# geekuillaume/node-speex-resampler

Hardware: AMD Instinct MI355X
Metric: input Msamples/s int16 44100->48000 q=7 2ch (whole job) (higher is better)
Workload: dtype f32

## Files before the change

### node-speex-resampler_amd/csrc/gen_fir_loop.py

```python
#!/usr/bin/env python3
import os

BANKS = {
    (10, 2): dict(A=[(28, 4), (36, 16)], B=[(52, 16), (68, 4)]),
    (5, 6): dict(A=[(4, 16), (20, 8), (28, 4), (36, 2)], B=[(40, 16), (56, 8), (64, 4), (38, 2)]),
    (5, 4): dict(A=[(28, 4), (36, 16)], B=[(52, 16), (68, 4)]),
}
SAMPLE_BASE = {10: 40, 5: 64}


def tap_reg(bank, t):
    for first, n in bank:
        if t < n:
            return first + t
        t -= n
    raise ValueError(t)


def bank_regs(bank):
    return [r for first, n in bank for r in range(first, first + n)]


class Variant:
    def __init__(self, R, S, CT, CF, padded, w16):
# ... 16 lines not shown
    def fma_bank(self, which, lo, hi):
        bank = self.banks[which]
        out = []
        for u in range(self.S):
            k = u if which == "A" else self.S + u
            for i in range(lo, hi):
                r = tap_reg(bank, u * self.R + i)
                h = r & 1
                p = r - h
                out.append("v_pk_fma_f32 %%[a%d], s[%d:%d], v[%d:%d], %%[a%d] op_sel:[%d,0,0] op_sel_hi:[%d,1,1]"
                           % (i, p, p + 1, self.pair(k), self.pair(k) + 1, i, h, h))
        return out

    def tap_loads(self, which, byte_off):
        out, t = [], 0
        for f, m in self.banks[which]:
            out.append("s_load_dword%s s[%d:%d], %%[rows], %%[off] offset:0x%x"
                       % ("x%d" % m if m > 1 else "", f, f + m - 1, byte_off + 4 * t))
            t += m
        return out

    def sample_reads(self, which, first_step):
        out = []
        if self.CT == 2 and not self.w16 and self.S % 2 == 0 and os.environ.get("SPEEXHIP_GEN_READ2"):
            for u in range(0, self.S, 2):
                k = u if which == "A" else self.S + u
                o0 = (first_step + u) * self.CF * 4 // 8
                o1 = (first_step + u + 1) * self.CF * 4 // 8
                p = self.pair(k)
                out.append("ds_read2_b64 v[%d:%d], %%[addr] offset0:%d offset1:%d" % (p, p + 3, o0, o1))
            return out
        for u in range(self.S):
            k = u if which == "A" else self.S + u
            o = (first_step + u) * self.CF * self.eb
            p = self.pair(k)
            if self.CT == 2 and not self.w16:
                out.append("ds_read_b64 v[%d:%d], %%[addr] offset:%d" % (p, p + 1, o))
            elif self.CT == 2:
                out.append("ds_read_b32 v%d, %%[addr] offset:%d" % (self.raw(k), o))
            elif not self.w16:
                out += ["ds_read_b32 v%d, %%[addr] offset:%d" % (p, o), "ds_read_b32 v%d, %%[addr2] offset:%d" % (p + 1, o)]
            else:
                out += ["ds_read_i16 v%d, %%[addr] offset:%d" % (p, o), "ds_read_i16 v%d, %%[addr2] offset:%d" % (p + 1, o)]
        return out

    def converts(self, which):
        if not self.w16:
            return []
        out = []
        for u in range(self.S):
            k = u if which == "A" else self.S + u
            p = self.pair(k)
            if self.CT == 2:
                out += ["v_cvt_f32_i32_sdwa v%d, sext(v%d) dst_sel:DWORD dst_unused:UNUSED_PAD src0_sel:WORD_0" % (p, self.raw(k)),
                        "v_cvt_f32_i32_sdwa v%d, sext(v%d) dst_sel:DWORD dst_unused:UNUSED_PAD src0_sel:WORD_1" % (p + 1, self.raw(k))]
            else:
                out += ["v_cvt_f32_i32_e32 v%d, v%d" % (p, p), "v_cvt_f32_i32_e32 v%d, v%d" % (p + 1, p + 1)]
        return out

    def loop(self, label, cnt, lo, hi):
        S, R = self.S, self.R
        bank_bytes = 4 * S * R
        adv = 2 * S * self.CF * self.eb
        body = ["s_sub_u32 %%[%s], %%[%s], 1" % (cnt, cnt), "s_cbranch_scc1 %d1f" % label, "%d0:" % label]
        body += ["s_waitcnt lgkmcnt(0)"] + self.tap_loads("B", bank_bytes) + self.sample_reads("B", S)
        body += self.converts("A") + self.fma_bank("A", lo, hi)
        body += ["s_waitcnt lgkmcnt(0)"]
        if self.padded:
            body += ["s_sub_u32 %[wrap], %[wrap], 1", "s_cmp_eq_u32 %[wrap], 0",
                     "s_cselect_b32 %[tmp], %[advpad], " + str(adv), "s_cselect_b32 %[wrap], %[wrapstep], %[wrap]",
                     "v_add_u32 %[addr], %[tmp], %[addr]"]
            if self.CT == 1:
                body += ["v_add_u32 %[addr2], %[tmp], %[addr2]"]
        else:
            body += ["v_add_u32 %%[addr], %d, %%[addr]" % adv]
            if self.CT == 1:
                body += ["v_add_u32 %%[addr2], %d, %%[addr2]" % adv]
        body += self.tap_loads("A", 2 * bank_bytes) + self.sample_reads("A", 0)
        body += self.converts("B") + self.fma_bank("B", lo, hi)
        body += ["s_add_u32 %%[off], %%[off], 0x%x" % (2 * bank_bytes), "s_sub_u32 %%[%s], %%[%s], 1" % (cnt, cnt),
                 "s_cbranch_scc0 %d0b" % label, "%d1:" % label]
        return body

    def lines(self):
        pro = self.tap_loads("A", 0) + self.sample_reads("A", 0)
        if self.R == 10:
            body = self.loop(1, "head", 0, 5) + self.loop(2, "main", 0, 10) + self.loop(3, "tail", 5, 10)
        else:
            body = self.loop(2, "main", 0, self.R)
        return pro + body + ["s_waitcnt lgkmcnt(0)"]

    def function(self):
        R = self.R
        asm = "\n".join('      "%s\\n"' % l for l in self.lines())
        outs = ['[a%d] "+v"(acc[%d])' % (i, i) for i in range(R)] + ['[addr] "+v"(addr)']
        if self.CT == 1:
            outs.append('[addr2] "+v"(addr2)')
        outs += ['[off] "+s"(off)', '[main] "+s"(main)']
        if R == 10:
            outs += ['[head] "+s"(head)', '[tail] "+s"(tail)']
        ins = ['[rows] "s"(rows_g)']
        if self.padded:
            outs += ['[wrap] "+s"(to_wrap)', '[tmp] "=&s"(tmp)']
            ins += ['[advpad] "s"(adv_pad)', '[wrapstep] "s"(wrap_step)']
        clob = ['"s%d"' % r for r in bank_regs(self.banks["A"]) + bank_regs(self.banks["B"])] + ['"v%d"' % r for r in self.vgprs()]
        return '''template <>
struct FirLoopAsm<%d, %d, %d, %s, %s> {
  static constexpr bool available = true;
  static constexpr int steps_per_bank = %d;
  // rows_g: the group's tap rows; addr / addr2: LDS byte addresses of the lane's first sample (second period);
  // head / main / tail: trips on rows [0, R/2) / all rows / rows [R/2, R); to_wrap, wrap_step: trips to the
  // first / between period boundaries of a padded window, adv_pad: window bytes per trip + the padding
  static __device__ __forceinline__ void run(f32x2 (&acc)[%d], const float *rows_g, uint32_t addr, uint32_t addr2,
                                             uint32_t head, uint32_t main, uint32_t tail, uint32_t to_wrap,
                                             uint32_t wrap_step, uint32_t adv_pad) {
    uint32_t off = 0, tmp;
    (void)tmp; (void)addr2; (void)head; (void)tail; (void)to_wrap; (void)wrap_step; (void)adv_pad;
    asm volatile(
%s
      : %s
      : %s
      : %s, "scc", "memory");
  }
};
''' % (R, self.CT, self.CF, "true" if self.padded else "false", "true" if self.w16 else "false", self.S, R, asm,
       ", ".join(outs), ", ".join(ins), ", ".join(clob))


class Variant64(Variant):

    def __init__(self, R, S, CT, CF, padded, w16=False):
        Variant.__init__(self, R, 2 * S, CT, CF, padded, False)
        self.S = S
        self.vbase = {10: 56, 5: 64}[R]
        self.w16 = w16
        self.eb = 2 if w16 else 4
        self.name = "A64_R%d_S%d_CT%d_CF%d_P%d_W%d" % (R, S, CT, CF, int(padded), int(w16))

    def quad(self, k):
        return self.vbase + 4 * k

    def vgprs(self):
        return list(range(self.vbase, self.vbase + 8 * self.S))

    def tap_pair(self, which, t):
        r = tap_reg(self.banks[which], 2 * t)
        assert r % 2 == 0 and tap_reg(self.banks[which], 2 * t + 1) == r + 1
        return r

    def fma_bank(self, which, lo, hi):
        out = []
        for u in range(self.S):
            k = u if which == "A" else self.S + u
            q = self.quad(k)
            for i in range(lo, hi):
                r = self.tap_pair(which, u * self.R + i)
                out.append("v_fma_f64 %%[a%dx], s[%d:%d], v[%d:%d], %%[a%dx]" % (i, r, r + 1, q, q + 1, i))
                out.append("v_fma_f64 %%[a%dy], s[%d:%d], v[%d:%d], %%[a%dy]" % (i, r, r + 1, q + 2, q + 3, i))
        return out

    def tap_loads(self, which, byte_off):
        out, t = [], 0
        for f, m in self.banks[which]:
            out.append("s_load_dword%s s[%d:%d], %%[rows], %%[off] offset:0x%x"
                       % ("x%d" % m if m > 1 else "", f, f + m - 1, byte_off + 4 * t))
            t += m
        return out

    def sample_reads(self, which, first_step):
        out = []
        for u in range(self.S):
            k = u if which == "A" else self.S + u
            o = (first_step + u) * self.CF * self.eb
# ... 144 lines not shown
        body += ["s_waitcnt lgkmcnt(0)"]
        if self.padded:
            body += ["s_sub_u32 %[wrap], %[wrap], 1", "s_cmp_eq_u32 %[wrap], 0",
                     "s_cselect_b32 %[tmp], %[advpad], " + str(adv), "s_cselect_b32 %[wrap], %[wrapstep], %[wrap]",
                     "v_add_u32 %[addr], %[tmp], %[addr]"]
        else:
            body += ["v_add_u32 %%[addr], %d, %%[addr]" % adv]
        body += self.tap_loads("A", 2 * bank_bytes) + self.sample_reads("A", 0)
        body += self.converts("B") + self.fma_bank("B", lo, hi)
        body += ["s_add_u32 %%[off], %%[off], 0x%x" % (2 * bank_bytes), "s_sub_u32 %%[%s], %%[%s], 1" % (cnt, cnt),
                 "s_cbranch_scc0 %d0b" % label, "%d1:" % label]
        return body

    def function(self):
        R = self.R
        asm = "\n".join('      "%s\\n"' % l for l in self.lines())
        outs = ['[a%d] "+v"(acc[%d])' % (i, i) for i in range(R)] + ['[addr] "+v"(addr)']
        outs += ['[off] "+s"(off)', '[main] "+s"(main)']
        if R == 10:
            outs += ['[head] "+s"(head)', '[tail] "+s"(tail)']
        ins = ['[rows] "s"(rows_g)']
        if self.padded:
            outs += ['[wrap] "+s"(to_wrap)', '[tmp] "=&s"(tmp)']
            ins += ['[advpad] "s"(adv_pad)', '[wrapstep] "s"(wrap_step)']
        clob = ['"s%d"' % r for r in bank_regs(self.banks["A"]) + bank_regs(self.banks["B"])] + ['"v%d"' % r for r in self.vgprs()]
        return '''template <>
struct FirLoopAsmPP<%d, %d, %s, %s> {
  static constexpr bool available = true;
  static constexpr int steps_per_bank = %d;
  // as FirLoopAsm::run; acc[i] = phases 2i and 2i + 1 of the lane's period; rows_g: [trip][step][2R] floats
  static __device__ __forceinline__ void run(f32x2 (&acc)[%d], const float *rows_g, uint32_t addr, uint32_t head, uint32_t main,
                                             uint32_t tail, uint32_t to_wrap, uint32_t wrap_step, uint32_t adv_pad) {
    uint32_t off = 0, tmp;
    (void)tmp; (void)head; (void)tail; (void)to_wrap; (void)wrap_step; (void)adv_pad;
    asm volatile(
%s
      : %s
      : %s
      : %s, "scc", "memory");
  }
};
''' % (R, self.CF, "true" if self.padded else "false", "true" if self.w16 else "false", self.S, R, asm,
       ", ".join(outs), ", ".join(ins), ", ".join(clob))

    def lines(self):
        pro = self.tap_loads("A", 0) + self.sample_reads("A", 0)
        if self.R == 10:
            body = self.loop(1, "head", 0, 5) + self.loop(2, "main", 0, 10) + self.loop(3, "tail", 5, 10)
        else:
            body = self.loop(2, "main", 0, self.R)
        return pro + body + ["s_waitcnt lgkmcnt(0)"]


def variants_pp():
    out = []
    for CF in (1, 2, 3):
        for w16 in (False, True):
            for padded in (False, True):
                out.append(VariantPP(10, 1, CF, padded, w16))
            out.append(VariantPP(5, R5_STEPS // 2, CF, False, w16))
    return out


def variants64():
    out = []
    for w16 in (False, True):
        for CT, CF in ((2, 2), (2, 4), (2, 6), (2, 8), (1, 1), (1, 3), (1, 5), (1, 7)):
            for padded in (False, True):
                out.append(Variant64(10, 1, CT, CF, padded, w16))
            out.append(Variant64(5, R5_STEPS // 2, CT, CF, False, w16))
    return out


def variants():
    out = []
    for w16 in (False, True):
        for CT, CF in ((2, 2), (2, 4), (2, 6), (2, 8), (1, 1), (1, 3), (1, 5), (1, 7), (2, 10), (2, 12), (2, 16)):
            for padded in (False, True):
                out.append(Variant(10, 2, CT, CF, padded, w16))
            out.append(Variant(5, R5_STEPS, CT, CF, False, w16))
    return out


R5_STEPS = 6

HEAD = '''// csrc/fir_loop_asm.inc -- GENERATED by csrc/gen_fir_loop.py; do not edit (see that file for the why and the how).
// The FIR inner loop of the period kernel as gfx950 ISA, one specialisation per (phases per wave, channels
// per lane, floats per frame, padded window, int16 window).  Included by kernels_period.hip only.

// primary template: no ISA variant for this layout -> fir_group runs its C++ loop
template <int R, int CT, int CF, bool PADDED, bool W16>
struct FirLoopAsm {
  static constexpr bool available = false;
};

'''


HEAD64 = '''
// ---- fp64 accumulator (round 4; gen_fir_loop.py, Variant64) ----
template <int R, int CT, int CF, bool PADDED, bool W16 = false>
struct FirLoopAsm64 {
  static constexpr bool available = false;
};

'''


HEADPP = '''
// ---- phase pairs: lane = (period, channel), two phases per packed FMA (round 4; gen_fir_loop.py, VariantPP) ----
template <int R, int CF, bool PADDED, bool W16>
struct FirLoopAsmPP {
  static constexpr bool available = false;
};

'''


def main():
    src = (HEAD + "\n".join(v.function() for v in variants()) + HEAD64 + "\n".join(v.function() for v in variants64()) +
           HEADPP + "\n".join(v.function() for v in variants_pp()))
    path = os.path.join(os.path.dirname(os.path.abspath(__file__)), "fir_loop_asm.inc")
    open(path, "w").write(src)
    print("wrote %s: %d + %d + %d variants, %d lines" % (path, len(variants()), len(variants64()), len(variants_pp()), src.count("\n")))


if __name__ == "__main__":
    main()
```

### node-speex-resampler_amd/csrc/kernels_period_impl.h

```cpp
#pragma once
#include <hip/hip_runtime.h>

#include <algorithm>
#include <cmath>
#include <cstdio>
#include <cstdlib>
#include <cstring>
#include <type_traits>
#include <vector>

#include "device_helpers.h"
#include "device_types.h"
#include "filter_design.h"
#include "kernels.h"

namespace speexhip {
#ifdef SPEEXHIP_STAMPS
static __device__ unsigned long long g_stamps[8192 * 16];
#define STAMP(k)                                                                                         \
  do {                                                                                                   \
    const uint32_t lin_ = blockIdx.x + gridDim.x * (blockIdx.y + gridDim.y * blockIdx.z);                \
    if ((threadIdx.x & 63u) == 0 && lin_ < 8192)                                                         \
      atomicMax(&g_stamps[lin_ * 16 + (k)], (unsigned long long)__builtin_amdgcn_s_memrealtime());        \
  } while (0)
#define STAMP_FIRST(k)                                                                                   \
  do {                                                                                                   \
    const uint32_t lin_ = blockIdx.x + gridDim.x * (blockIdx.y + gridDim.y * blockIdx.z);                \
    if ((threadIdx.x & 63u) == 0 && lin_ < 8192)                                                         \
      atomicMax(&g_stamps[lin_ * 16 + (k)], ~(unsigned long long)__builtin_amdgcn_s_memrealtime());       \
  } while (0)
#else
#define STAMP(k) do { } while (0)
#define STAMP_FIRST(k) do { } while (0)
#endif
namespace {

typedef float f32x2 __attribute__((ext_vector_type(2)));
__host__ __device__ constexpr int bank_taps(int r) { return r == 10 ? 20 : 30; }
typedef uint32_t u32x4_a4 __attribute__((ext_vector_type(4), aligned(4)));
typedef uint32_t u32x2_a4 __attribute__((ext_vector_type(2), aligned(4)));
typedef __attribute__((address_space(1))) u32x4_a4 g_u32x4_a4;
typedef __attribute__((address_space(1))) u32x2_a4 g_u32x2_a4;
typedef float f32x4_a4 __attribute__((ext_vector_type(4), aligned(4)));
typedef float f32x2_a4 __attribute__((ext_vector_type(2), aligned(4)));

__device__ __forceinline__ void fma_tap(f32x2 &acc, const f32x2 &tap_pair, const f32x2 &x, bool hi) {
  if (hi)
    asm("v_pk_fma_f32 %0, %1, %2, %0 op_sel:[1,0,0] op_sel_hi:[1,1,1]" : "+v"(acc) : "s"(tap_pair), "v"(x));
  else
    asm("v_pk_fma_f32 %0, %1, %2, %0 op_sel:[0,0,0] op_sel_hi:[0,1,1]" : "+v"(acc) : "s"(tap_pair), "v"(x));
}

#include "fir_loop_asm.inc"

__device__ __forceinline__ void set_fir_priority(const PeriodParams &p) {
  if (p.prio & 4u) {
    const uint32_t tg_id = (__builtin_amdgcn_s_getreg(4 | (16 << 6) | (3 << 11)));
    if (tg_id & 1u) {
      __builtin_amdgcn_s_setprio(1);
      return;
    }
  }
  __builtin_amdgcn_s_setprio(0);
}

struct LaneCtx {
  uint32_t C;
  uint32_t cg;
  bool live;
  bool live_b;
  uint32_t xlane;
  uint64_t K_lane;
};

template <int CT, bool ONE_GROUP, bool PADDED, int CGF = 0, bool PP = false, bool ROWS = false>
__device__ __forceinline__ LaneCtx lane_ctx(const PeriodParams &p, uint32_t xshift, uint32_t m_lo,
                                            uint32_t m_cnt, uint32_t lane) {
  constexpr uint32_t kGroups = ONE_GROUP ? 1u : static_cast<uint32_t>(CGF);
  const uint32_t cgroups = kGroups != 0 ? kGroups : p.cgroups;
  LaneCtx c;
  c.C = kGroups != 0 ? kGroups * CT : p.channels;
  static_assert(!ROWS || (CGF == 4 && CT == 2), "the row mapping is for frames of four channel pairs");
  c.cg = ONE_GROUP ? 0 : ROWS ? lane >> 4 : lane % cgroups;
  const uint32_t pl = ONE_GROUP ? lane : ROWS ? (lane & 15u) : lane / cgroups;
  const uint32_t lane_max = (CT == 1 && !PP) ? p.half_periods : p.lane_periods;
  c.live = pl < lane_max && pl < m_cnt;
  c.live_b = CT == 1 && !PP && pl < lane_max && pl + p.half_periods < m_cnt;
  c.xlane = xshift + min(pl, lane_max - 1) * (p.num * c.C + (PADDED ? p.pad : 0u)) + c.cg * CT;
  c.K_lane = static_cast<uint64_t>(m_lo + pl) * p.den;
  return c;
}

template <int R, int CT, bool PADDED, int CF = 0, bool W16 = false>
__device__ __forceinline__ void fir_group(const PeriodParams &p, const float *__restrict__ rows, const float *xs,
                                          const LaneCtx &c, uint32_t g, bool skip_all, f32x2 (&acc)[R]) {
  const uint32_t C = c.C;
  const uint32_t delta_g = p.delta[g];
  using E = typename std::conditional<W16, int16_t, float>::type;
  const E *xp = reinterpret_cast<const E *>(xs) + c.xlane + delta_g * C;
#ifndef SPEEXHIP_CXX_FIR_LOOP
  constexpr bool kIsa16 = W16 && CF != 0 && FirLoopAsm<R, CT, CF, PADDED, W16>::available;
#else
  constexpr bool kIsa16 = false;
#endif
  if constexpr (kIsa16) {
    using Isa = FirLoopAsm<R, CT, CF, PADDED, true>;
    constexpr uint32_t kStepsPerTrip = 2 * Isa::steps_per_bank;
    const uint32_t trips = skip_all ? 0u : p.delta[2 * p.groups + g];
    const uint32_t head = R == 10 ? trips & 15u : 0u, tail = R == 10 ? (trips >> 4) & 15u : 0u;
    const float *rows_g = rows + static_cast<size_t>(g) * p.l4 * (2 * bank_taps(R));
    const uint32_t addr = static_cast<uint32_t>(reinterpret_cast<uintptr_t>(xs)) + (c.xlane + delta_g * C) * 2u;
    auto sgpr = [](uint32_t v) { return static_cast<uint32_t>(__builtin_amdgcn_readfirstlane(static_cast<int>(v))); };
    const uint64_t rows_bits = reinterpret_cast<uint64_t>(rows_g);
    const float *rows_s = reinterpret_cast<const float *>(static_cast<uint64_t>(sgpr(static_cast<uint32_t>(rows_bits))) |
                                                          static_cast<uint64_t>(sgpr(static_cast<uint32_t>(rows_bits >> 32))) << 32);
    Isa::run(acc, rows_s, addr, CT == 1 ? addr + p.half_offset * 2u : 0u, sgpr(head), sgpr((trips >> 8) - head - tail),
             sgpr(tail), sgpr(PADDED ? p.delta[p.groups + g] : 0u), sgpr(p.wrap_step),
             sgpr((kStepsPerTrip * CF + p.pad) * 2u));
    return;
  }
#ifndef SPEEXHIP_CXX_FIR_LOOP
  using Isa = FirLoopAsm<R, CT, CF, PADDED, false>;
  if constexpr (!W16 && CF != 0 && Isa::available) {
    constexpr uint32_t kStepsPerTrip = 2 * Isa::steps_per_bank;
    static_assert(kStepsPerTrip * R == 2 * bank_taps(R), "the ISA loop and the tap rows disagree on the trip");
    const uint32_t trips = skip_all ? 0u : p.delta[2 * p.groups + g];
    const uint32_t head = R == 10 ? trips & 15u : 0u, tail = R == 10 ? (trips >> 4) & 15u : 0u;
    const float *rows_g = rows + static_cast<size_t>(g) * p.l4 * (2 * bank_taps(R));
    const uint32_t addr = static_cast<uint32_t>(reinterpret_cast<uintptr_t>(xp));
    auto sgpr = [](uint32_t v) { return static_cast<uint32_t>(__builtin_amdgcn_readfirstlane(static_cast<int>(v))); };
    const uint64_t rows_bits = reinterpret_cast<uint64_t>(rows_g);
    const float *rows_s = reinterpret_cast<const float *>(static_cast<uint64_t>(sgpr(static_cast<uint32_t>(rows_bits))) |
                                                          static_cast<uint64_t>(sgpr(static_cast<uint32_t>(rows_bits >> 32))) << 32);
    Isa::run(acc, rows_s, addr, CT == 1 ? addr + p.half_offset * 4u : 0u, sgpr(head), sgpr((trips >> 8) - head - tail),
             sgpr(tail), sgpr(PADDED ? p.delta[p.groups + g] : 0u), sgpr(p.wrap_step),
             sgpr((kStepsPerTrip * CF + p.pad) * 4u));
// ... 502 lines not shown
  auto params = [&]() -> PeriodParams {
    if constexpr (kReload) return load_k(pp);
    return p0;
  };
  constexpr bool kRows = PADDED && CGF == 4 && !W16 && AM == 0;
  const LaneCtx c = lane_ctx<CT, ONE_GROUP, PADDED, CGF, AM == 2, kRows>(p0, xshift, m_lo, m_cnt, lane);
  const uint32_t g_step = p0.wave_groups * nsplit;
  uint32_t g = zsplit * p0.wave_groups + wave;
  if (g >= p0.groups) return;
  PeriodParams p = p0;
  for (;;) {
    f32x2 acc[R];
#pragma unroll
    for (int i = 0; i < R; i++) acc[i] = f32x2{0.f, 0.f};
#ifdef SPEEXHIP_STAMPS
    const unsigned long long fir_t0 = __builtin_amdgcn_s_memtime(), fir_r0 = __builtin_amdgcn_s_memrealtime();
#endif
    if constexpr (AM == 2) {
      fir_group_pp<R, ONE_GROUP ? 1 : CGF, PADDED, W16>(p, rows, xs, c, g, SPEEXHIP_DIAG_SKIP(p, 4u), 0u, 1u, acc);
    } else if constexpr (AM == 1) {
      double acc64[R][2];
#pragma unroll
      for (int i = 0; i < R; i++) acc64[i][0] = acc64[i][1] = 0.0;
      fir_group64<R, CT, PADDED, ONE_GROUP ? CT : CT * CGF, W16>(p, reinterpret_cast<const double *>(rows), xs, c, g,
                                                                SPEEXHIP_DIAG_SKIP(p, 4u), 0u, 1u, acc64);
#pragma unroll
      for (int i = 0; i < R; i++) acc[i] = f32x2{static_cast<float>(acc64[i][0]), static_cast<float>(acc64[i][1])};
    } else {
      fir_group<R, CT, PADDED, ONE_GROUP ? CT : CT * CGF, W16>(p, rows, xs, c, g, SPEEXHIP_DIAG_SKIP(p, 4u), acc);
    }
#ifdef SPEEXHIP_STAMPS
    {
      asm volatile("" ::"v"(acc[0]));
      const unsigned long long fir_t1 = __builtin_amdgcn_s_memtime(), fir_r1 = __builtin_amdgcn_s_memrealtime();
      const uint32_t lin_ = blockIdx.x + gridDim.x * (blockIdx.y + gridDim.y * blockIdx.z);
      if ((threadIdx.x & 63u) == 0 && lin_ < 8192) atomicMax(&g_stamps[lin_ * 16 + 7], fir_t1 - fir_t0);
      if (threadIdx.x == 0 && lin_ < 8192) {
        g_stamps[lin_ * 16 + 9] = fir_t1 - fir_t0;
        g_stamps[lin_ * 16 + 10] = fir_r1 - fir_r0;
      }
    }
#endif
    STAMP(5);
    const PeriodParams q = params();
    if constexpr (kRows && sizeof(T) == 2 && R == 10) {
      if (!SPEEXHIP_DIAG_SKIP(q, 8u)) {
        StreamDesc d;
        if constexpr (kReload)
          d = load_k(dp);
        else
          d = d0;
        if (q.prio & 2u) __builtin_amdgcn_s_setprio(2);
        store_group_rows<R>(q, d, c, g, c.live, acc);
        if (q.prio & 2u) set_fir_priority(q);
        STAMP(6);
      }
    } else if (!SPEEXHIP_DIAG_SKIP(q, 8u) && c.live) {
      StreamDesc d;
      if constexpr (kReload)
        d = load_k(dp);
      else
        d = d0;
      if (q.prio & 2u) __builtin_amdgcn_s_setprio(2);
      if constexpr (AM == 2)
        store_group_pp<R, ONE_GROUP ? 1 : CGF, T>(q, d, c, g, acc);
      else
        store_group<R, CT, ONE_GROUP, T>(q, d, c, g, acc);
      if (q.prio & 2u) set_fir_priority(q);
      STAMP(6);
    }
    g += g_step;
    if (g >= q.groups) return;
    p = q;
  }
}

template <typename T>
struct StagedImage {
  static constexpr uint32_t kRowDwords = 16 * 5 * (sizeof(T) == 4 ? 2 : 1) + 1;
  static constexpr uint32_t kBytes = 64 * kRowDwords * 4;
  static constexpr uint32_t kAt = (kStagedLdsBytes - kBytes) / 16 * 16;
};

template <int R, int CT, typename T>
__device__ __forceinline__ void fir_tile_staged(const PeriodParams &p0, KParams pp, const float *__restrict__ rows, KDesc dp,
                                                float *xs, uint32_t xshift, uint32_t m_lo, uint32_t m_cnt, uint32_t wave,
                                                uint32_t lane, uint32_t zsplit) {
  static_assert(R == 5 && CT == 2, "written for stereo groups of five phases");
  using Img = StagedImage<T>;
  constexpr uint32_t kDpf = sizeof(T) == 4 ? 2u : 1u;
  uint32_t *img = reinterpret_cast<uint32_t *>(reinterpret_cast<char *>(xs) + Img::kAt);
  const uint32_t g = zsplit * p0.wave_groups + wave;
  if (wave < p0.wave_groups && g < p0.groups) {
    const LaneCtx c = lane_ctx<CT, true, false>(p0, xshift, m_lo, m_cnt, lane);
    f32x2 acc[R];
#pragma unroll
    for (int i = 0; i < R; i++) acc[i] = f32x2{0.f, 0.f};
    fir_group<R, CT, false, CT, false>(p0, rows, xs, c, g, SPEEXHIP_DIAG_SKIP(p0, 4u), acc);
    uint32_t *row = img + lane * Img::kRowDwords + wave * (R * kDpf);
#pragma unroll
    for (int i = 0; i < R; i++) {
      if constexpr (sizeof(T) == 4) {
        row[2 * i] = __float_as_uint(acc[i].x);
        row[2 * i + 1] = __float_as_uint(acc[i].y);
      } else {
        row[i] = round_pack_pcm(acc[i].x, acc[i].y);
      }
    }
  }
  __syncthreads();
  const PeriodParams q = load_k(pp);
  const StreamDesc d = load_k(dp);
  if (SPEEXHIP_DIAG_SKIP(q, 8u)) return;
  if (q.prio & 2u) __builtin_amdgcn_s_setprio(2);
  constexpr uint32_t kFb = 4u * kDpf;
  const uint32_t ph_lo = zsplit * q.wave_groups * R;
  const uint32_t ph_n = ph_lo < q.den ? min(q.wave_groups * R, q.den - ph_lo) : 0u;
  const uint32_t pieces = (ph_n * kFb + 15u) / 16u + 1u;
  const uint64_t out = reinterpret_cast<uint64_t>(d.out);
#pragma clang loop unroll(disable)
  for (uint32_t t = threadIdx.x; t < m_cnt * pieces; t += q.threads) {
    const uint32_t r = t / pieces, k = t - r * pieces;
    const int64_t f0 = static_cast<int64_t>(m_lo + r) * q.den + ph_lo - d.k_shift;
    const int64_t f_lo = max(f0, static_cast<int64_t>(0));
    const int64_t f_hi = min(f0 + static_cast<int64_t>(ph_n), static_cast<int64_t>(d.n_out));
    if (f_lo >= f_hi) continue;
    const uint64_t a_lo = out + static_cast<uint64_t>(f_lo) * kFb, a_hi = out + static_cast<uint64_t>(f_hi) * kFb;
    const uint64_t blk = (a_lo & ~static_cast<uint64_t>(15)) + 16u * k;
    if (blk >= a_hi) continue;
    const uint64_t s = max(blk, a_lo), e = min(blk + 16u, a_hi);
    const uint32_t col = static_cast<uint32_t>((static_cast<int64_t>(s - out) - f0 * kFb) >> 2);
    const uint32_t *src = img + r * Img::kRowDwords + col;
    if (e - s == 16u) {
      const u32x4 v = u32x4{src[0], src[1], src[2], src[3]};
#ifdef SPEEXHIP_DIAG
      if (SPEEXHIP_DIAG_SKIP(q, 256u)) {
        *reinterpret_cast<G<u32x4> *>(blk) = v;
        continue;
      }
      if (SPEEXHIP_DIAG_SKIP(q, 512u)) {
        asm volatile("global_store_dwordx4 %0, %1, off sc1" ::"v"(blk), "v"(v) : "memory");
        continue;
      }
#endif
      __builtin_nontemporal_store(v, reinterpret_cast<G<u32x4> *>(blk));
    } else {
#pragma unroll
      for (uint32_t j = 0; j < 3; j++)
        if (s + 4u * j < e) reinterpret_cast<g_u32 *>(s)[j] = src[j];
    }
  }
}

template <int R, int CT, bool PADDED, int CF, bool W16>
__device__ __forceinline__ void fir_group_part(const PeriodParams &p, const float *__restrict__ rows, const float *xs,
                                               const LaneCtx &c, uint32_t g, uint32_t part, uint32_t parts,
                                               f32x2 (&acc)[R]) {
  using Isa = FirLoopAsm<R, CT, CF, PADDED, W16>;
  static_assert(CF != 0 && Isa::available, "tap-range shares run the ISA loop");
  constexpr uint32_t kStepsPerTrip = 2 * Isa::steps_per_bank;
  constexpr uint32_t EB = W16 ? 2u : 4u;
  auto sgpr = [](uint32_t v) { return static_cast<uint32_t>(__builtin_amdgcn_readfirstlane(static_cast<int>(v))); };
  const uint32_t delta_g = p.delta[g];
  const uint32_t trips = SPEEXHIP_DIAG_SKIP(p, 4u) ? 0u : p.delta[2 * p.groups + g];
  const uint32_t head = R == 10 ? trips & 15u : 0u, tail = R == 10 ? (trips >> 4) & 15u : 0u, total = trips >> 8;
  const uint32_t t0 = sgpr(total * part / parts), t1 = sgpr(total * (part + 1) / parts);
  auto overlap = [&](uint32_t lo, uint32_t hi) {
    const uint32_t a = max(t0, lo), b = min(t1, hi);
    return b > a ? b - a : 0u;
  };
  const uint32_t main_end = total - tail;
  uint32_t wraps = 0, to_wrap = 0;
  if constexpr (PADDED) {
    const uint32_t to_wrap0 = p.delta[p.groups + g];
    to_wrap = to_wrap0;
    if (to_wrap0 != 0 && t0 >= to_wrap0) {
      const uint32_t past = t0 - to_wrap0;
      wraps = 1 + past / p.wrap_step;
      to_wrap = p.wrap_step - past % p.wrap_step;
    } else if (to_wrap0 != 0) {
      to_wrap = to_wrap0 - t0;
    }
  }
  const float *rows_g = rows + (static_cast<size_t>(g) * p.l4 + t0) * (2 * bank_taps(R));
  const uint32_t addr = static_cast<uint32_t>(reinterpret_cast<uintptr_t>(xs)) +
                        ((c.xlane + delta_g * c.C) + t0 * kStepsPerTrip * CF + wraps * p.pad) * EB;
  const uint64_t rows_bits = reinterpret_cast<uint64_t>(rows_g);
  const float *rows_s = reinterpret_cast<const float *>(static_cast<uint64_t>(sgpr(static_cast<uint32_t>(rows_bits))) |
                                                        static_cast<uint64_t>(sgpr(static_cast<uint32_t>(rows_bits >> 32))) << 32);
  Isa::run(acc, rows_s, addr, CT == 1 ? addr + p.half_offset * EB : 0u, sgpr(overlap(0, head)), sgpr(overlap(head, main_end)),
           sgpr(overlap(main_end, total)), sgpr(to_wrap), sgpr(p.wrap_step), sgpr((kStepsPerTrip * CF + p.pad) * EB));
}

template <int R, int CT, bool ONE_GROUP, bool PADDED, typename T, int CGF = 0, bool W16 = false, bool PP = false>
__device__ __forceinline__ void fir_tile_parts(KParams pp, const float *__restrict__ rows, KDesc dp, float *xs,
// ... 79 lines not shown
    wg = p.wave_groups;
    parts = p.ksplit;
    part = 0;
    gw = wave;
    while (gw >= wg) {
      gw -= wg;
      part++;
    }
    g = zsplit * wg + gw;
    valid = g < p.groups;
    if (valid) fir_group64<R, CT, PADDED, CF, W16>(p, rows, xs, c, g, SPEEXHIP_DIAG_SKIP(p, 4u), part, parts, acc);
  }
  __syncthreads();
  double *sums = reinterpret_cast<double *>(xs);
  if (valid && part != 0) {
    double *mine = sums + (static_cast<size_t>(part - 1) * wg + gw) * (2 * R * 64) + lane;
#pragma unroll
    for (int i = 0; i < R; i++) {
      mine[(2 * i) * 64] = acc[i][0];
      mine[(2 * i + 1) * 64] = acc[i][1];
    }
  }
  __syncthreads();
  if (!valid || part != 0) return;
  for (uint32_t j = 1; j < parts; j++) {
    const double *theirs = sums + (static_cast<size_t>(j - 1) * wg + gw) * (2 * R * 64) + lane;
#pragma unroll
    for (int i = 0; i < R; i++) {
      acc[i][0] += theirs[(2 * i) * 64];
      acc[i][1] += theirs[(2 * i + 1) * 64];
    }
  }
  const PeriodParams q = load_k(pp);
  if (SPEEXHIP_DIAG_SKIP(q, 8u) || !c.live) return;
  const StreamDesc d = load_k(dp);
  f32x2 out[R];
#pragma unroll
  for (int i = 0; i < R; i++) out[i] = f32x2{static_cast<float>(acc[i][0]), static_cast<float>(acc[i][1])};
  store_group<R, CT, ONE_GROUP, T>(q, d, c, g, out);
}

template <int R>
__device__ __forceinline__ void touch_rows(const PeriodParams &p, const float *__restrict__ rows, uint32_t &sink) {
  if (p.touch == 0) return;
  const uint32_t bytes = p.groups * p.l4 * static_cast<uint32_t>(2 * bank_taps(R) * 4);
#pragma clang loop unroll(disable)
  for (uint32_t off = threadIdx.x * 128u; off < bytes; off += p.threads * 128u)
    asm volatile("global_load_dword %0, %1, %2" : "+v"(sink) : "v"(off), "s"(rows) : "memory");
}

template <int R, int CT, bool ONE_GROUP, bool PADDED, typename T, int CGF = 0, bool W16 = false, bool KS = false, int AM = 0,
          bool ST = false>
__global__ __launch_bounds__(1024, (R == 10 && !KS) ? 8 : 4) __attribute__((amdgpu_num_sgpr(80))) void resample_period(
    PeriodParams p, const float *__restrict__ rows, DescPack pack) {
  extern __shared__ __attribute__((aligned(16))) float xs[];
  __builtin_amdgcn_s_setprio(3);
  STAMP(0);
#ifdef SPEEXHIP_STAMPS
  {
    const uint32_t lin_ = blockIdx.x + gridDim.x * (blockIdx.y + gridDim.y * blockIdx.z);
    if (threadIdx.x == 0 && lin_ < 8192)
      g_stamps[lin_ * 16 + 8] = (static_cast<unsigned long long>(__builtin_amdgcn_s_getreg(20 | (0 << 6) | (31 << 11))) << 32) |
                                __builtin_amdgcn_s_getreg(4 | (0 << 6) | (31 << 11));
  }
#endif
  const StreamDesc d = pack.d[blockIdx.y];
  if (!(p.prio & 1u)) __builtin_amdgcn_s_setprio(0);
  const uint32_t m_total = d.m_total;
  const uint32_t m_lo = blockIdx.x * p.lane_periods;
  const uint32_t m_cnt = m_lo < m_total ? min(p.lane_periods, m_total - m_lo) : 1u;
  WindowGeom wg;
  if (!window_geom_plain<T>(d, p.channels, p.num, p.tail_frames, m_lo, m_cnt, p.threads, PADDED ? p.pad : 0u,
                            PADDED ? p.period_magic : 0u, &wg))
    wg = window_geom<T>(d, p.channels, p.num, p.tail_frames, m_lo, m_cnt, p.threads, PADDED ? p.pad : 0u,
                        PADDED ? p.period_magic : 0u);
  if (SPEEXHIP_DIAG_SKIP(p, 64u)) return;
  if (blockIdx.x == p.history_block) {
    if (blockIdx.z == 0) roll_history<T>(p.channels, d, p.threads);
    return;
  }
  if (d.n_out == 0 || blockIdx.x > p.history_block || m_lo >= m_total) return;
  STAMP(1);
  uint32_t row_sink = 0;
  if (!SPEEXHIP_DIAG_SKIP(p, 2u)) {
    constexpr int UNR = PADDED ? 3 : (sizeof(T) == 4 ? (ONE_GROUP ? 5 : 3) : 5);
    u32x4 w[UNR];
    bool plain = false, plain_padded = false;
    if constexpr (!PADDED) plain = window_is_plain<UNR, T>(wg);
    if constexpr (PADDED && !W16) plain_padded = window_is_plain_padded<UNR, T>(wg);
    if (plain_padded) {
      window_fetch_plain<UNR, T>(wg, w);
      STAMP(2);
      window_commit_plain_padded<UNR, T>(xs, wg, w);
    } else if (plain) {
      window_fetch_plain<UNR, T>(wg, w);
      STAMP(2);
      if constexpr (W16)
        window_commit_plain16<UNR>(reinterpret_cast<int16_t *>(xs), wg, w);
      else
        window_commit_plain<UNR, T>(xs, wg, w);
    } else {
      window_fetch<UNR, T>(wg, w);
      STAMP(2);
      if constexpr (W16)
        window_commit16<UNR>(reinterpret_cast<int16_t *>(xs), d, wg, w);
      else
        window_commit<UNR, T>(xs, d, wg, w);
    }
#ifndef SPEEXHIP_CXX_FIR_LOOP
    if constexpr (AM != 0 || FirLoopAsm<R, CT, ONE_GROUP ? CT : CT * CGF, PADDED, W16>::available) touch_rows<R>(p, rows, row_sink);
#endif
    asm volatile("s_waitcnt vmcnt(0)" ::: "memory");
    asm volatile("" ::"v"(row_sink));
  }
  STAMP(3);
  __syncthreads();
  if (p.prio & 7u) set_fir_priority(p);
  STAMP(4);
  if (SPEEXHIP_DIAG_SKIP(p, 128u)) return;
  const uint32_t wave = __builtin_amdgcn_readfirstlane(threadIdx.x >> 6);
  if constexpr (KS) {
    const __attribute__((address_space(4))) KernArgs *ka =
        (const __attribute__((address_space(4))) KernArgs *)__builtin_amdgcn_kernarg_segment_ptr();
    const KDesc dp = &ka->pack.d[blockIdx.y];
    if constexpr (AM == 1)
      fir_tile_parts64<R, CT, ONE_GROUP, PADDED, T, CGF, W16>(&ka->p, reinterpret_cast<const double *>(rows), dp, xs, wg.xshift,
                                                              m_lo, m_cnt, wave, threadIdx.x & 63u, blockIdx.z);
    else
      fir_tile_parts<R, CT, ONE_GROUP, PADDED, T, CGF, W16, AM == 2>(&ka->p, rows, dp, xs, wg.xshift, m_lo, m_cnt, wave,
                                                                    threadIdx.x & 63u, blockIdx.z);
    return;
  } else if constexpr (ST) {
    static_assert(ONE_GROUP && !PADDED && !W16 && AM == 0, "staged stores: stereo frames on the float window");
    const __attribute__((address_space(4))) KernArgs *ka =
        (const __attribute__((address_space(4))) KernArgs *)__builtin_amdgcn_kernarg_segment_ptr();
    fir_tile_staged<R, CT, T>(p, &ka->p, rows, &ka->pack.d[blockIdx.y], xs, wg.xshift, m_lo, m_cnt, wave, threadIdx.x & 63u,
                              blockIdx.z);
  } else {
  if (wave >= p.wave_groups) return;
  const __attribute__((address_space(4))) KernArgs *ka =
      (const __attribute__((address_space(4))) KernArgs *)__builtin_amdgcn_kernarg_segment_ptr();
  const KDesc dp = &ka->pack.d[blockIdx.y];
  fir_tile<R, CT, ONE_GROUP, PADDED, T, CGF, W16, AM>(p, d, &ka->p, rows, dp, xs, wg.xshift, m_lo, m_cnt, wave,
                                                  threadIdx.x & 63u, blockIdx.z, gridDim.z);
  }
}

template <int R, int CT, bool ONE_GROUP, bool PADDED, typename T, int CGF = 0, bool W16 = false, bool KS = false, int AM = 0,
          bool ST = false>
hipError_t launch_rc(const PeriodParams &p, const DescPack *pack, dim3 grid, uint32_t threads, size_t lds_bytes,
                     hipStream_t stream) {
#ifdef SPEEXHIP_CXX_FIR_LOOP
  constexpr bool kParts = false;
#else
  constexpr bool kParts = KS && (AM != 0 || FirLoopAsm<R, CT, ONE_GROUP ? CT : CT * CGF, PADDED, W16>::available);
#endif
  if constexpr (KS && !kParts) {
    return hipErrorInvalidValue;
  } else {
    static std::atomic<uint64_t> seen{0};
    opt_in_lds_on_this_device(resample_period<R, CT, ONE_GROUP, PADDED, T, CGF, W16, KS, AM, ST>, seen);
    hipLaunchKernelGGL((resample_period<R, CT, ONE_GROUP, PADDED, T, CGF, W16, KS, AM, ST>), grid, dim3(threads), lds_bytes, stream,
                       p, p.rows, *pack);
    return hipGetLastError();
  }
}

}
}
```

Measured before the change: 184,600.

## Move staging barrier inside FIR ISA loop to overlap tap loads

For the staged stereo path, the workgroup barrier after the window staging now sits inside a new hand-written ISA entry of the FIR loop. The first tap bank's scalar loads and the per-group delta/trip table loads are issued before the barrier, so their latency overlaps the wait for other waves. The table lookups are also hoisted into the window fetch phase, and a barrier is added after loading the kernel params. The change adds another generated asm variant and restructures barrier placement, so a barrier count mismatch between waves could deadlock.

```diff
diff --git a/node-speex-resampler_amd/csrc/fir_loop_barrier_asm.inc b/node-speex-resampler_amd/csrc/fir_loop_barrier_asm.inc
--- /dev/null
+++ b/node-speex-resampler_amd/csrc/fir_loop_barrier_asm.inc
@@ -0,0 +1,121 @@
+
+template <int R, int CT, int CF, bool PADDED, bool W16>
+struct FirLoopBarrierAsm {
+  static constexpr bool available = false;
+};
+
+template <>
+struct FirLoopBarrierAsm<5, 2, 2, false, false> {
+  static constexpr bool available = true;
+  static constexpr int steps_per_bank = 6;
+  static __device__ __forceinline__ void run(f32x2 (&acc)[5], const float *rows_g, uint32_t addr, uint32_t main) {
+    uint32_t off = 0;
+    asm volatile(
+      "s_load_dwordx16 s[4:19], %[rows], %[off] offset:0x0\n"
+      "s_load_dwordx8 s[20:27], %[rows], %[off] offset:0x40\n"
+      "s_load_dwordx4 s[28:31], %[rows], %[off] offset:0x60\n"
+      "s_load_dwordx2 s[36:37], %[rows], %[off] offset:0x70\n"
+      "s_waitcnt vmcnt(0) lgkmcnt(0)\n"
+      "s_barrier\n"
+      "ds_read_b64 v[64:65], %[addr] offset:0\n"
+      "ds_read_b64 v[66:67], %[addr] offset:8\n"
+      "ds_read_b64 v[68:69], %[addr] offset:16\n"
+      "ds_read_b64 v[70:71], %[addr] offset:24\n"
+      "ds_read_b64 v[72:73], %[addr] offset:32\n"
+      "ds_read_b64 v[74:75], %[addr] offset:40\n"
+      "s_sub_u32 %[main], %[main], 1\n"
+      "s_cbranch_scc1 21f\n"
+      "20:\n"
+      "s_waitcnt lgkmcnt(0)\n"
+      "s_load_dwordx16 s[40:55], %[rows], %[off] offset:0x78\n"
+      "s_load_dwordx8 s[56:63], %[rows], %[off] offset:0xb8\n"
+      "s_load_dwordx4 s[64:67], %[rows], %[off] offset:0xd8\n"
+      "s_load_dwordx2 s[38:39], %[rows], %[off] offset:0xe8\n"
+      "ds_read_b64 v[76:77], %[addr] offset:48\n"
+      "ds_read_b64 v[78:79], %[addr] offset:56\n"
+      "ds_read_b64 v[80:81], %[addr] offset:64\n"
+      "ds_read_b64 v[82:83], %[addr] offset:72\n"
+      "ds_read_b64 v[84:85], %[addr] offset:80\n"
+      "ds_read_b64 v[86:87], %[addr] offset:88\n"
+      "v_pk_fma_f32 %[a0], s[4:5], v[64:65], %[a0] op_sel:[0,0,0] op_sel_hi:[0,1,1]\n"
+      "v_pk_fma_f32 %[a1], s[4:5], v[64:65], %[a1] op_sel:[1,0,0] op_sel_hi:[1,1,1]\n"
+      "v_pk_fma_f32 %[a2], s[6:7], v[64:65], %[a2] op_sel:[0,0,0] op_sel_hi:[0,1,1]\n"
+      "v_pk_fma_f32 %[a3], s[6:7], v[64:65], %[a3] op_sel:[1,0,0] op_sel_hi:[1,1,1]\n"
+      "v_pk_fma_f32 %[a4], s[8:9], v[64:65], %[a4] op_sel:[0,0,0] op_sel_hi:[0,1,1]\n"
+      "v_pk_fma_f32 %[a0], s[8:9], v[66:67], %[a0] op_sel:[1,0,0] op_sel_hi:[1,1,1]\n"
+      "v_pk_fma_f32 %[a1], s[10:11], v[66:67], %[a1] op_sel:[0,0,0] op_sel_hi:[0,1,1]\n"
+      "v_pk_fma_f32 %[a2], s[10:11], v[66:67], %[a2] op_sel:[1,0,0] op_sel_hi:[1,1,1]\n"
+      "v_pk_fma_f32 %[a3], s[12:13], v[66:67], %[a3] op_sel:[0,0,0] op_sel_hi:[0,1,1]\n"
+      "v_pk_fma_f32 %[a4], s[12:13], v[66:67], %[a4] op_sel:[1,0,0] op_sel_hi:[1,1,1]\n"
+      "v_pk_fma_f32 %[a0], s[14:15], v[68:69], %[a0] op_sel:[0,0,0] op_sel_hi:[0,1,1]\n"
+      "v_pk_fma_f32 %[a1], s[14:15], v[68:69], %[a1] op_sel:[1,0,0] op_sel_hi:[1,1,1]\n"
+      "v_pk_fma_f32 %[a2], s[16:17], v[68:69], %[a2] op_sel:[0,0,0] op_sel_hi:[0,1,1]\n"
+      "v_pk_fma_f32 %[a3], s[16:17], v[68:69], %[a3] op_sel:[1,0,0] op_sel_hi:[1,1,1]\n"
+      "v_pk_fma_f32 %[a4], s[18:19], v[68:69], %[a4] op_sel:[0,0,0] op_sel_hi:[0,1,1]\n"
+      "v_pk_fma_f32 %[a0], s[18:19], v[70:71], %[a0] op_sel:[1,0,0] op_sel_hi:[1,1,1]\n"
+      "v_pk_fma_f32 %[a1], s[20:21], v[70:71], %[a1] op_sel:[0,0,0] op_sel_hi:[0,1,1]\n"
+      "v_pk_fma_f32 %[a2], s[20:21], v[70:71], %[a2] op_sel:[1,0,0] op_sel_hi:[1,1,1]\n"
+      "v_pk_fma_f32 %[a3], s[22:23], v[70:71], %[a3] op_sel:[0,0,0] op_sel_hi:[0,1,1]\n"
+      "v_pk_fma_f32 %[a4], s[22:23], v[70:71], %[a4] op_sel:[1,0,0] op_sel_hi:[1,1,1]\n"
+      "v_pk_fma_f32 %[a0], s[24:25], v[72:73], %[a0] op_sel:[0,0,0] op_sel_hi:[0,1,1]\n"
+      "v_pk_fma_f32 %[a1], s[24:25], v[72:73], %[a1] op_sel:[1,0,0] op_sel_hi:[1,1,1]\n"
+      "v_pk_fma_f32 %[a2], s[26:27], v[72:73], %[a2] op_sel:[0,0,0] op_sel_hi:[0,1,1]\n"
+      "v_pk_fma_f32 %[a3], s[26:27], v[72:73], %[a3] op_sel:[1,0,0] op_sel_hi:[1,1,1]\n"
+      "v_pk_fma_f32 %[a4], s[28:29], v[72:73], %[a4] op_sel:[0,0,0] op_sel_hi:[0,1,1]\n"
+      "v_pk_fma_f32 %[a0], s[28:29], v[74:75], %[a0] op_sel:[1,0,0] op_sel_hi:[1,1,1]\n"
+      "v_pk_fma_f32 %[a1], s[30:31], v[74:75], %[a1] op_sel:[0,0,0] op_sel_hi:[0,1,1]\n"
+      "v_pk_fma_f32 %[a2], s[30:31], v[74:75], %[a2] op_sel:[1,0,0] op_sel_hi:[1,1,1]\n"
+      "v_pk_fma_f32 %[a3], s[36:37], v[74:75], %[a3] op_sel:[0,0,0] op_sel_hi:[0,1,1]\n"
+      "v_pk_fma_f32 %[a4], s[36:37], v[74:75], %[a4] op_sel:[1,0,0] op_sel_hi:[1,1,1]\n"
+      "s_waitcnt lgkmcnt(0)\n"
+      "v_add_u32 %[addr], 96, %[addr]\n"
+      "s_load_dwordx16 s[4:19], %[rows], %[off] offset:0xf0\n"
+      "s_load_dwordx8 s[20:27], %[rows], %[off] offset:0x130\n"
+      "s_load_dwordx4 s[28:31], %[rows], %[off] offset:0x150\n"
+      "s_load_dwordx2 s[36:37], %[rows], %[off] offset:0x160\n"
+      "ds_read_b64 v[64:65], %[addr] offset:0\n"
+      "ds_read_b64 v[66:67], %[addr] offset:8\n"
+      "ds_read_b64 v[68:69], %[addr] offset:16\n"
+      "ds_read_b64 v[70:71], %[addr] offset:24\n"
+      "ds_read_b64 v[72:73], %[addr] offset:32\n"
+      "ds_read_b64 v[74:75], %[addr] offset:40\n"
+      "v_pk_fma_f32 %[a0], s[40:41], v[76:77], %[a0] op_sel:[0,0,0] op_sel_hi:[0,1,1]\n"
+      "v_pk_fma_f32 %[a1], s[40:41], v[76:77], %[a1] op_sel:[1,0,0] op_sel_hi:[1,1,1]\n"
+      "v_pk_fma_f32 %[a2], s[42:43], v[76:77], %[a2] op_sel:[0,0,0] op_sel_hi:[0,1,1]\n"
+      "v_pk_fma_f32 %[a3], s[42:43], v[76:77], %[a3] op_sel:[1,0,0] op_sel_hi:[1,1,1]\n"
+      "v_pk_fma_f32 %[a4], s[44:45], v[76:77], %[a4] op_sel:[0,0,0] op_sel_hi:[0,1,1]\n"
+      "v_pk_fma_f32 %[a0], s[44:45], v[78:79], %[a0] op_sel:[1,0,0] op_sel_hi:[1,1,1]\n"
+      "v_pk_fma_f32 %[a1], s[46:47], v[78:79], %[a1] op_sel:[0,0,0] op_sel_hi:[0,1,1]\n"
+      "v_pk_fma_f32 %[a2], s[46:47], v[78:79], %[a2] op_sel:[1,0,0] op_sel_hi:[1,1,1]\n"
+      "v_pk_fma_f32 %[a3], s[48:49], v[78:79], %[a3] op_sel:[0,0,0] op_sel_hi:[0,1,1]\n"
+      "v_pk_fma_f32 %[a4], s[48:49], v[78:79], %[a4] op_sel:[1,0,0] op_sel_hi:[1,1,1]\n"
+      "v_pk_fma_f32 %[a0], s[50:51], v[80:81], %[a0] op_sel:[0,0,0] op_sel_hi:[0,1,1]\n"
+      "v_pk_fma_f32 %[a1], s[50:51], v[80:81], %[a1] op_sel:[1,0,0] op_sel_hi:[1,1,1]\n"
+      "v_pk_fma_f32 %[a2], s[52:53], v[80:81], %[a2] op_sel:[0,0,0] op_sel_hi:[0,1,1]\n"
+      "v_pk_fma_f32 %[a3], s[52:53], v[80:81], %[a3] op_sel:[1,0,0] op_sel_hi:[1,1,1]\n"
+      "v_pk_fma_f32 %[a4], s[54:55], v[80:81], %[a4] op_sel:[0,0,0] op_sel_hi:[0,1,1]\n"
+      "v_pk_fma_f32 %[a0], s[54:55], v[82:83], %[a0] op_sel:[1,0,0] op_sel_hi:[1,1,1]\n"
+      "v_pk_fma_f32 %[a1], s[56:57], v[82:83], %[a1] op_sel:[0,0,0] op_sel_hi:[0,1,1]\n"
+      "v_pk_fma_f32 %[a2], s[56:57], v[82:83], %[a2] op_sel:[1,0,0] op_sel_hi:[1,1,1]\n"
+      "v_pk_fma_f32 %[a3], s[58:59], v[82:83], %[a3] op_sel:[0,0,0] op_sel_hi:[0,1,1]\n"
+      "v_pk_fma_f32 %[a4], s[58:59], v[82:83], %[a4] op_sel:[1,0,0] op_sel_hi:[1,1,1]\n"
+      "v_pk_fma_f32 %[a0], s[60:61], v[84:85], %[a0] op_sel:[0,0,0] op_sel_hi:[0,1,1]\n"
+      "v_pk_fma_f32 %[a1], s[60:61], v[84:85], %[a1] op_sel:[1,0,0] op_sel_hi:[1,1,1]\n"
+      "v_pk_fma_f32 %[a2], s[62:63], v[84:85], %[a2] op_sel:[0,0,0] op_sel_hi:[0,1,1]\n"
+      "v_pk_fma_f32 %[a3], s[62:63], v[84:85], %[a3] op_sel:[1,0,0] op_sel_hi:[1,1,1]\n"
+      "v_pk_fma_f32 %[a4], s[64:65], v[84:85], %[a4] op_sel:[0,0,0] op_sel_hi:[0,1,1]\n"
+      "v_pk_fma_f32 %[a0], s[64:65], v[86:87], %[a0] op_sel:[1,0,0] op_sel_hi:[1,1,1]\n"
+      "v_pk_fma_f32 %[a1], s[66:67], v[86:87], %[a1] op_sel:[0,0,0] op_sel_hi:[0,1,1]\n"
+      "v_pk_fma_f32 %[a2], s[66:67], v[86:87], %[a2] op_sel:[1,0,0] op_sel_hi:[1,1,1]\n"
+      "v_pk_fma_f32 %[a3], s[38:39], v[86:87], %[a3] op_sel:[0,0,0] op_sel_hi:[0,1,1]\n"
+      "v_pk_fma_f32 %[a4], s[38:39], v[86:87], %[a4] op_sel:[1,0,0] op_sel_hi:[1,1,1]\n"
+      "s_add_u32 %[off], %[off], 0xf0\n"
+      "s_sub_u32 %[main], %[main], 1\n"
+      "s_cbranch_scc0 20b\n"
+      "21:\n"
+      "s_waitcnt lgkmcnt(0)\n"
+      : [a0] "+v"(acc[0]), [a1] "+v"(acc[1]), [a2] "+v"(acc[2]), [a3] "+v"(acc[3]), [a4] "+v"(acc[4]), [addr] "+v"(addr), [off] "+s"(off), [main] "+s"(main)
+      : [rows] "s"(rows_g)
+      : "s4", "s5", "s6", "s7", "s8", "s9", "s10", "s11", "s12", "s13", "s14", "s15", "s16", "s17", "s18", "s19", "s20", "s21", "s22", "s23", "s24", "s25", "s26", "s27", "s28", "s29", "s30", "s31", "s36", "s37", "s40", "s41", "s42", "s43", "s44", "s45", "s46", "s47", "s48", "s49", "s50", "s51", "s52", "s53", "s54", "s55", "s56", "s57", "s58", "s59", "s60", "s61", "s62", "s63", "s64", "s65", "s66", "s67", "s38", "s39", "v64", "v65", "v66", "v67", "v68", "v69", "v70", "v71", "v72", "v73", "v74", "v75", "v76", "v77", "v78", "v79", "v80", "v81", "v82", "v83", "v84", "v85", "v86", "v87", "scc", "memory");
+  }
+};
diff --git a/node-speex-resampler_amd/csrc/gen_fir_loop.py b/node-speex-resampler_amd/csrc/gen_fir_loop.py
--- a/node-speex-resampler_amd/csrc/gen_fir_loop.py
+++ b/node-speex-resampler_amd/csrc/gen_fir_loop.py
@@ -122,13 +122,37 @@
                  "s_cbranch_scc0 %d0b" % label, "%d1:" % label]
         return body
 
-    def lines(self):
-        pro = self.tap_loads("A", 0) + self.sample_reads("A", 0)
+    def lines(self, barrier=False):
+        mid = ["s_waitcnt vmcnt(0) lgkmcnt(0)", "s_barrier"] if barrier else []
+        pro = self.tap_loads("A", 0) + mid + self.sample_reads("A", 0)
         if self.R == 10:
             body = self.loop(1, "head", 0, 5) + self.loop(2, "main", 0, 10) + self.loop(3, "tail", 5, 10)
         else:
             body = self.loop(2, "main", 0, self.R)
         return pro + body + ["s_waitcnt lgkmcnt(0)"]
+
+    def barrier_function(self):
+        assert self.R == 5 and not self.padded and self.CT == 2
+        asm = "\n".join('      "%s\\n"' % l for l in self.lines(True))
+        outs = ['[a%d] "+v"(acc[%d])' % (i, i) for i in range(self.R)] + ['[addr] "+v"(addr)', '[off] "+s"(off)', '[main] "+s"(main)']
+        clob = ['"s%d"' % r for r in bank_regs(self.banks["A"]) + bank_regs(self.banks["B"])] + ['"v%d"' % r for r in self.vgprs()]
+        return '''template <>
+struct FirLoopBarrierAsm<%d, %d, %d, %s, %s> {
+  static constexpr bool available = true;
+  static constexpr int steps_per_bank = %d;
+  // FirLoopAsm::run for a wave that has NOT yet passed the barrier behind the window's staging: the barrier is in here,
+  // between the first tap bank's loads and the first sample reads (a trip count of 0 still passes it)
+  static __device__ __forceinline__ void run(f32x2 (&acc)[%d], const float *rows_g, uint32_t addr, uint32_t main) {
+    uint32_t off = 0;
+    asm volatile(
+%s
+      : %s
+      : [rows] "s"(rows_g)
+      : %s, "scc", "memory");
+  }
+};
+''' % (self.R, self.CT, self.CF, "true" if self.padded else "false", "true" if self.w16 else "false", self.S, self.R, asm,
+       ", ".join(outs), ", ".join(clob))
 
     def function(self):
         R = self.R
@@ -439,6 +463,10 @@
     return out
 
 
+def variants_barrier():
+    return [Variant(5, R5_STEPS, 2, 2, False, False)]
+
+
 R5_STEPS = 6
 
 HEAD = '''// csrc/fir_loop_asm.inc -- GENERATED by csrc/gen_fir_loop.py; do not edit (see that file for the why and the how).
@@ -472,6 +500,23 @@
 };
 
 '''
+
+
+HEADBARRIER = '''// csrc/fir_loop_barrier_asm.inc -- GENERATED by csrc/gen_fir_loop.py; do not edit (see that file for the why and the how).
+// The entry of the period kernel's FIR loop with the staging barrier inside it (Variant.lines(barrier=True)): included by
+// kernels_period_impl.h behind fir_loop_asm.inc.
+
+// primary template: no barrier entry for this layout
+template <int R, int CT, int CF, bool PADDED, bool W16>
+struct FirLoopBarrierAsm {
+  static constexpr bool available = false;
+};
+
+'''
+
+
+def barrier_source():
+    return HEADBARRIER + "\n".join(v.barrier_function() for v in variants_barrier())
 
 
 def main():
@@ -480,6 +525,9 @@
     path = os.path.join(os.path.dirname(os.path.abspath(__file__)), "fir_loop_asm.inc")
     open(path, "w").write(src)
     print("wrote %s: %d + %d + %d variants, %d lines" % (path, len(variants()), len(variants64()), len(variants_pp()), src.count("\n")))
+    path = os.path.join(os.path.dirname(os.path.abspath(__file__)), "fir_loop_barrier_asm.inc")
+    open(path, "w").write(barrier_source())
+    print("wrote %s: %d variants" % (path, len(variants_barrier())))
 
 
 if __name__ == "__main__":
diff --git a/node-speex-resampler_amd/csrc/kernels_period_impl.h b/node-speex-resampler_amd/csrc/kernels_period_impl.h
--- a/node-speex-resampler_amd/csrc/kernels_period_impl.h
+++ b/node-speex-resampler_amd/csrc/kernels_period_impl.h
@@ -52,6 +52,7 @@
 }
 
 #include "fir_loop_asm.inc"
+#include "fir_loop_barrier_asm.inc"
 
 __device__ __forceinline__ void set_fir_priority(const PeriodParams &p) {
   if (p.prio & 4u) {
@@ -720,21 +721,56 @@
   static constexpr uint32_t kAt = (kStagedLdsBytes - kBytes) / 16 * 16;
 };
 
+struct StagedGroup {
+  uint32_t delta_g;
+  uint32_t trips;
+};
+#if defined(SPEEXHIP_CXX_FIR_LOOP) || defined(SPEEXHIP_STAMPS)
+constexpr bool kBarrierEntry = false;
+#else
+constexpr bool kBarrierEntry = true;
+#endif
+
 template <int R, int CT, typename T>
 __device__ __forceinline__ void fir_tile_staged(const PeriodParams &p0, KParams pp, const float *__restrict__ rows, KDesc dp,
                                                 float *xs, uint32_t xshift, uint32_t m_lo, uint32_t m_cnt, uint32_t wave,
-                                                uint32_t lane, uint32_t zsplit) {
+                                                uint32_t lane, uint32_t zsplit, const StagedGroup &sg) {
   static_assert(R == 5 && CT == 2, "written for stereo groups of five phases");
   using Img = StagedImage<T>;
   constexpr uint32_t kDpf = sizeof(T) == 4 ? 2u : 1u;
   uint32_t *img = reinterpret_cast<uint32_t *>(reinterpret_cast<char *>(xs) + Img::kAt);
   const uint32_t g = zsplit * p0.wave_groups + wave;
+  if (SPEEXHIP_DIAG_SKIP(p0, 128u)) {
+    __syncthreads();
+    return;
+  }
+  if constexpr (!kBarrierEntry) {
+    __syncthreads();
+    STAMP(4);
+  }
   if (wave < p0.wave_groups && g < p0.groups) {
     const LaneCtx c = lane_ctx<CT, true, false>(p0, xshift, m_lo, m_cnt, lane);
     f32x2 acc[R];
 #pragma unroll
     for (int i = 0; i < R; i++) acc[i] = f32x2{0.f, 0.f};
-    fir_group<R, CT, false, CT, false>(p0, rows, xs, c, g, SPEEXHIP_DIAG_SKIP(p0, 4u), acc);
+#ifndef SPEEXHIP_CXX_FIR_LOOP
+    if constexpr (kBarrierEntry) {
+      using Isa = FirLoopBarrierAsm<R, CT, CT, false, false>;
+      static_assert(Isa::available && 2 * Isa::steps_per_bank * R == 2 * bank_taps(R),
+                    "the staged launch enters the ISA loop of its layout through the barrier");
+      auto sgpr = [](uint32_t v) { return static_cast<uint32_t>(__builtin_amdgcn_readfirstlane(static_cast<int>(v))); };
+      const uint32_t trips = SPEEXHIP_DIAG_SKIP(p0, 4u) ? 0u : sg.trips >> 8;
+      const float *rows_g = rows + static_cast<size_t>(g) * p0.l4 * (2 * bank_taps(R));
+      const uint32_t addr = static_cast<uint32_t>(reinterpret_cast<uintptr_t>(xs + c.xlane + sg.delta_g * c.C));
+      const uint64_t rows_bits = reinterpret_cast<uint64_t>(rows_g);
+      const float *rows_s = reinterpret_cast<const float *>(static_cast<uint64_t>(sgpr(static_cast<uint32_t>(rows_bits))) |
+                                                            static_cast<uint64_t>(sgpr(static_cast<uint32_t>(rows_bits >> 32))) << 32);
+      Isa::run(acc, rows_s, addr, sgpr(trips));
+    } else
+#endif
+    {
+      fir_group<R, CT, false, CT, false>(p0, rows, xs, c, g, SPEEXHIP_DIAG_SKIP(p0, 4u), acc);
+    }
     uint32_t *row = img + lane * Img::kRowDwords + wave * (R * kDpf);
 #pragma unroll
     for (int i = 0; i < R; i++) {
@@ -745,10 +781,12 @@
         row[i] = round_pack_pcm(acc[i].x, acc[i].y);
       }
     }
-  }
-  __syncthreads();
+  } else if constexpr (kBarrierEntry) {
+    __syncthreads();
+  }
   const PeriodParams q = load_k(pp);
   const StreamDesc d = load_k(dp);
+  __syncthreads();
   if (SPEEXHIP_DIAG_SKIP(q, 8u)) return;
   if (q.prio & 2u) __builtin_amdgcn_s_setprio(2);
   constexpr uint32_t kFb = 4u * kDpf;
@@ -994,6 +1032,21 @@
   if (d.n_out == 0 || blockIdx.x > p.history_block || m_lo >= m_total) return;
   STAMP(1);
   uint32_t row_sink = 0;
+  [[maybe_unused]] uint32_t st_wave = 0;
+  [[maybe_unused]] StagedGroup sg{0u, 0u};
+  [[maybe_unused]] auto group_tables = [&]() {
+    if constexpr (ST) {
+      const uint32_t gs = min(blockIdx.z * p.wave_groups + st_wave, p.groups - 1u);
+      const __attribute__((address_space(4))) uint32_t *tab = (const __attribute__((address_space(4))) uint32_t *)p.delta;
+      sg.delta_g = tab[gs];
+      sg.trips = tab[2 * p.groups + gs];
+      asm volatile("" : "+s"(sg.delta_g), "+s"(sg.trips));
+    }
+  };
+  if constexpr (ST) {
+    st_wave = __builtin_amdgcn_readfirstlane(threadIdx.x >> 6);
+    if (SPEEXHIP_DIAG_SKIP(p, 2u)) group_tables();
+  }
   if (!SPEEXHIP_DIAG_SKIP(p, 2u)) {
     constexpr int UNR = PADDED ? 3 : (sizeof(T) == 4 ? (ONE_GROUP ? 5 : 3) : 5);
     u32x4 w[UNR];
@@ -1007,6 +1060,7 @@
     } else if (plain) {
       window_fetch_plain<UNR, T>(wg, w);
       STAMP(2);
+      group_tables();
       if constexpr (W16)
         window_commit_plain16<UNR>(reinterpret_cast<int16_t *>(xs), wg, w);
       else
@@ -1014,6 +1068,7 @@
     } else {
       window_fetch<UNR, T>(wg, w);
       STAMP(2);
+      group_tables();
       if constexpr (W16)
         window_commit16<UNR>(reinterpret_cast<int16_t *>(xs), d, wg, w);
       else
@@ -1026,6 +1081,15 @@
     asm volatile("" ::"v"(row_sink));
   }
   STAMP(3);
+  if constexpr (ST) {
+    static_assert(ONE_GROUP && !PADDED && !W16 && AM == 0 && !KS, "staged stores: stereo frames on the float window");
+    if (p.prio & 7u) set_fir_priority(p);
+    const __attribute__((address_space(4))) KernArgs *ka =
+        (const __attribute__((address_space(4))) KernArgs *)__builtin_amdgcn_kernarg_segment_ptr();
+    fir_tile_staged<R, CT, T>(p, &ka->p, rows, &ka->pack.d[blockIdx.y], xs, wg.xshift, m_lo, m_cnt, st_wave, threadIdx.x & 63u,
+                              blockIdx.z, sg);
+    return;
+  }
   __syncthreads();
   if (p.prio & 7u) set_fir_priority(p);
   STAMP(4);
@@ -1042,12 +1106,6 @@
       fir_tile_parts<R, CT, ONE_GROUP, PADDED, T, CGF, W16, AM == 2>(&ka->p, rows, dp, xs, wg.xshift, m_lo, m_cnt, wave,
                                                                     threadIdx.x & 63u, blockIdx.z);
     return;
-  } else if constexpr (ST) {
-    static_assert(ONE_GROUP && !PADDED && !W16 && AM == 0, "staged stores: stereo frames on the float window");
-    const __attribute__((address_space(4))) KernArgs *ka =
-        (const __attribute__((address_space(4))) KernArgs *)__builtin_amdgcn_kernarg_segment_ptr();
-    fir_tile_staged<R, CT, T>(p, &ka->p, rows, &ka->pack.d[blockIdx.y], xs, wg.xshift, m_lo, m_cnt, wave, threadIdx.x & 63u,
-                              blockIdx.z);
   } else {
   if (wave >= p.wave_groups) return;
   const __attribute__((address_space(4))) KernArgs *ka =
```

New measurement: 185,600 (median of 4 runs). Within noise of the previous version (+0.6%).
